# CliffKai/BridgeLang

Hardware: AMD Instinct MI355X
Metric: action-seqs/sec (7-DoF, 224px) openvla-7b bf16 (higher is better)
Workload: dtype bf16; 1 GPU; openvla-7b bf16 inference (BASELINE configs[1]): batch 16 synthetic 224px frames + 32-token prompts per GPU, predict_action = vision towers + projector + Llama prefill S=288 + 6 cached decode steps, greedy; 7 batches in flight: per step one batch is submitted (vision+prefill) while decode iteration g of the batch submitted g steps earlier, g = 1..6, runs as ONE merged 96-row pass over the weights ; batch_per_gpu=16, prompt_len=32, seq_len=288, replicas=1, hip_graph=True, pipeline_depth=7

## Files before the change

### bridgelang_amd/csrc/gemm_bf16.hip

```cpp
#include "gemm_common.h"
#include <stdlib.h>

namespace bl_gemm_bf16_impl {
using namespace blgemm;

typedef __attribute__((ext_vector_type(4))) short s16x4_t;

template <int EPI>
__global__ __launch_bounds__(256) void gemm128_kernel(GemmArgs p) {
#if defined(__HIP_DEVICE_COMPILE__)
  constexpr int BM = 128, BN = 128, WN = 2, NWAVE = 4;
  constexpr int TM = 64, TN = 64, MT = 4, NT = 4;
  constexpr int A_BYTES = BM * ROW_BYTES, BUF_BYTES = A_BYTES + BN * ROW_BYTES;
  extern __shared__ __attribute__((aligned(16))) char smem[];

  int tm, tn;
  tile_coords(p, tm, tn);
  const int m0 = tm * BM, n0 = tn * BN;
  const int tid = threadIdx.x, lane = tid & 63;
  const int wave = __builtin_amdgcn_readfirstlane(tid >> 6);
  const int wm = wave / WN, wn = wave % WN;
  const int kt32 = p.K >> 5;

  const unsigned a_bytes = (unsigned)min((long)p.M * p.lda * 2, 0xffffffffL);
// ... 382 lines not shown
        }
      }
    }
    asm volatile("s_waitcnt lgkmcnt(0)" ::: "memory");
    __builtin_amdgcn_s_barrier();
  }
#undef BL_STAGE
#undef BL_WAIT_TILES
  if constexpr (SK > 0) {
    float* slab = p.slab + (long)blockIdx.y * p.M * p.N;
#pragma unroll
    for (int i = 0; i < NB; ++i)
#pragma unroll
      for (int j = 0; j < MB; ++j) {
        const int m = wave * 16 * MB + j * 16 + l15, n = n0 + i * 16 + lg * 4;
        if (gridDim.y == 1) epilogue_store4<EPI>(p, m, n, acc[i][j]);
        else if (m < p.M && n < p.N) *(f32x4_t*)(slab + (long)m * p.N + n) = acc[i][j];
      }
    return;
  }
  if (p.splitk > 1) {
    float* slab = p.slab + (long)blockIdx.y * p.M * p.N;
#pragma unroll
    for (int i = 0; i < NB; ++i)
#pragma unroll
      for (int j = 0; j < MB; ++j) {
        const int m = wave * 16 * MB + j * 16 + l15, n = n0 + i * 16 + lg * 4;
        if (m < p.M && n < p.N) *(f32x4_t*)(slab + (long)m * p.N + n) = acc[i][j];
      }
    return;
  }
#pragma unroll
  for (int i = 0; i < NB; ++i)
#pragma unroll
    for (int j = 0; j < MB; ++j)
      epilogue_store4<EPI>(p, wave * 16 * MB + j * 16 + l15, n0 + i * 16 + lg * 4, acc[i][j]);
#endif
}

template <int EPI, int NWV, int SK>
__global__ __launch_bounds__(NWV * 64) void gemm_rows_stream_kernel(GemmArgs p, int n_tiles) {
#if defined(__HIP_DEVICE_COMPILE__)
  constexpr int MR = 6, GS = 4, NWB = 4;
  constexpr int KT_BYTES = MR * 16 * ROW_BYTES, XBUF = 2 * KT_BYTES;
  constexpr int XP = 24 / NWV, OPS = XP + GS;
  static_assert(24 % NWV == 0 && XP <= GS, "the chunk's 24 LDS-DMA pieces are dealt evenly to the waves, one per k-step");
  constexpr int LV = SK >= 8 ? 3 : SK >= 4 ? 2 : SK >= 2 ? 1 : 0;
  extern __shared__ __attribute__((aligned(16))) char smem[];
  const int tid = threadIdx.x, lane = tid & 63;
  const int wave = __builtin_amdgcn_readfirstlane(tid >> 6);
  const int l15 = lane & 15, lg = lane >> 4;
  const int tile_raw = (int)blockIdx.x * NWV + wave;
  const bool live = tile_raw < n_tiles;
  const int tile = live ? tile_raw : n_tiles - 1;
  const int kt32 = p.K >> 5;
  const int ks0 = (int)blockIdx.y * SK * p.fold_ks, nks = SK * p.fold_ks;
  const int NC = (nks + GS - 1) / GS;

  const unsigned a_bytes = (unsigned)min((long)p.M * p.lda * 2, 0xffffffffL);
  const __amdgpu_buffer_rsrc_t rsA = __builtin_amdgcn_make_buffer_rsrc((void*)p.A, 0, a_bytes, 0x00020000);
  const int prow = lane >> 3, pchunk = (lane & 7) ^ prow;
  unsigned voffA[XP];
  int ldsA[XP];
#pragma unroll
  for (int j = 0; j < XP; ++j) {
    const int q = j * NWV + wave, kt = q / 12, rb = q - kt * 12;
    voffA[j] = (unsigned)(((long)(rb * 8 + prow) * p.lda) * 2 + kt * 128 + pchunk * 16);
    ldsA[j] = kt * KT_BYTES + rb * 1024;
  }
  const u32x4_t* wbase = (const u32x4_t*)p.W + ((long)tile * kt32 + ks0) * 64 + lane;
  u32x4_t wbuf[NWB][GS];

#define BL_RS_ISSUE_PART(SLOT, C, J)                                                                          \
  do {                                                                                                        \
    const int cc__ = min((C), NC - 1);                                                                        \
    if ((J) < XP) BL_GLDS(rsA, smem + (SLOT) * XBUF + ldsA[(J) < XP ? (J) : 0], voffA[(J) < XP ? (J) : 0], (ks0 + cc__ * GS) * 64); \
    wbuf[SLOT][J] = __builtin_nontemporal_load(wbase + (long)min(cc__ * GS + (J), nks - 1) * 64);             \
  } while (0)
#define BL_RS_READX(DST, XB, S)                                                                               \
  do {                                                                                                        \
    const char* xs__ = (XB) + ((S) >> 1) * KT_BYTES + offA + ((c0 ^ (((S) & 1) * 4)) << 4);                    \
    _Pragma("unroll") for (int j = 0; j < MR; ++j) DST[j] = *(const bf16x8_t*)(xs__ + j * 16 * ROW_BYTES);    \
  } while (0)
#define BL_RS_FOLD_LEVEL(L)                                                                \
  if constexpr (LV > L) {                                                                   \
    if (!parked) {                                                                          \
      if (!((sl >> L) & 1)) {                                                               \
        _Pragma("unroll") for (int j = 0; j < MR; ++j) hold[L][j] = acc[j];                 \
        parked = true;                                                                      \
      } else {                                                                              \
        _Pragma("unroll") for (int j = 0; j < MR; ++j) acc[j] = hold[L][j] + acc[j];        \
      }                                                                                     \
    }                                                                                       \
  }
#define BL_RS_CHUNK(SLOT, C)                                                                                  \
  {                                                                                                           \
    asm volatile("s_waitcnt vmcnt(%0)" ::"n"(2 * OPS) : "memory");                                            \
    __builtin_amdgcn_s_barrier();                                                                             \
    const char* xb = smem + (SLOT) * XBUF;                                                                    \
    bf16x8_t xf[2][MR];                                                                                       \
    BL_RS_READX(xf[0], xb, 0);                                                                                \
    _Pragma("unroll") for (int s2 = 0; s2 < GS; ++s2) {                                                       \
      if (s2 + 1 < GS) BL_RS_READX(xf[(s2 + 1) & 1], xb, s2 + 1);                                             \
      __builtin_amdgcn_sched_barrier(0);    \
      const int kidx = (C) * GS + s2;                                                                         \
      if (kidx < nks) {                                                                                       \
        const bf16x8_t wf = __builtin_bit_cast(bf16x8_t, wbuf[SLOT][s2]);                                     \
        _Pragma("unroll") for (int j = 0; j < MR; ++j)                                                        \
          acc[j] = __builtin_amdgcn_mfma_f32_16x16x32_bf16(wf, xf[s2 & 1][j], acc[j], 0, 0, 0);               \
        if (SK > 1 && s2 == GS - 1 && kidx + 1 == fold_next) {           \
          bool parked = false;                                                                                \
              \
          _Pragma("unroll") for (int j = 0; j < MR; ++j) asm volatile("" : "+v"(acc[j]));                     \
          BL_RS_FOLD_LEVEL(0) BL_RS_FOLD_LEVEL(1) BL_RS_FOLD_LEVEL(2)                                         \
          if (parked) {                                                                                       \
            _Pragma("unroll") for (int j = 0; j < MR; ++j) acc[j] = (f32x4_t){0.f, 0.f, 0.f, 0.f};            \
          }                                                                                                   \
          fold_next += p.fold_ks;                                                                             \
          ++sl;                                                                                               \
        }                                                                                                     \
      }                                                                                                       \
      __builtin_amdgcn_sched_barrier(0);                                                                      \
      BL_RS_ISSUE_PART(((SLOT) + NWB - 1) % NWB, (C) + NWB - 1, s2);                                          \
      __builtin_amdgcn_sched_barrier(0);                                                                      \
    }                                                                                                         \
    asm volatile("s_waitcnt lgkmcnt(0)" ::: "memory");                                                        \
  }

  const int c0 = lg ^ (lane & 7);
  const int offA = l15 * ROW_BYTES;
  f32x4_t acc[MR], hold[LV ? LV : 1][MR];
#pragma unroll
  for (int j = 0; j < MR; ++j) acc[j] = (f32x4_t){0.f, 0.f, 0.f, 0.f};
  int fold_next = p.fold_ks, sl = 0;

#pragma unroll
  for (int c = 0; c < NWB - 1; ++c) {
#pragma unroll
    for (int j = 0; j < GS; ++j) BL_RS_ISSUE_PART(c, c, j);
    __builtin_amdgcn_sched_barrier(0);
  }
  for (int cb = 0; cb < NC; cb += NWB) {
    BL_RS_CHUNK(0, cb)
    BL_RS_CHUNK(1, cb + 1)
    BL_RS_CHUNK(2, cb + 2)
    BL_RS_CHUNK(3, cb + 3)
  }
#undef BL_RS_CHUNK
#undef BL_RS_FOLD_LEVEL
#undef BL_RS_READX
#undef BL_RS_ISSUE_PART
  if (!live) return;
  float* slab = p.slab + (long)blockIdx.y * p.M * p.N;
#pragma unroll
  for (int j = 0; j < MR; ++j) {
    const int m = j * 16 + l15, n = tile * 16 + lg * 4;
    if (gridDim.y == 1) epilogue_store4<EPI>(p, m, n, acc[j]);
    else if (m < p.M) *(f32x4_t*)(slab + (long)m * p.N + n) = acc[j];
  }
#endif
}

template <int EPI, int NT, int NST = 3>
__global__ __launch_bounds__(256) void gemm_mid2_kernel(GemmArgs p) {
#if defined(__HIP_DEVICE_COMPILE__)
  constexpr int BM = 160, BN = 32 * NT, MT = 5, LPS = 5 + NT;
  constexpr int A_BYTES = BM * ROW_BYTES, BUF_BYTES = A_BYTES + NT * 4096;
  extern __shared__ __attribute__((aligned(16))) char smem[];
  const int n0 = blockIdx.x * BN, m0 = blockIdx.y * BM;
  const int tid = threadIdx.x, lane = tid & 63;
  const int wave = __builtin_amdgcn_readfirstlane(tid >> 6);
  const int wm = wave >> 1, wn = wave & 1;
  const int kt32 = p.K >> 5;

  const unsigned a_bytes = (unsigned)min((long)p.M * p.lda * 2, 0xffffffffL);
  const unsigned w_bytes = (unsigned)min((long)p.N * p.K * 2, 0xffffffffL);
  const __amdgpu_buffer_rsrc_t rsA = __builtin_amdgcn_make_buffer_rsrc((void*)p.A, 0, a_bytes, 0x00020000);
  const __amdgpu_buffer_rsrc_t rsW = __builtin_amdgcn_make_buffer_rsrc((void*)p.W, 0, w_bytes, 0x00020000);

  const int prow = lane >> 3, pchunk = (lane & 7) ^ prow;
  unsigned voffA[MT];
#pragma unroll
  for (int j = 0; j < MT; ++j) voffA[j] = (unsigned)(((long)(m0 + (j * 4 + wave) * 8 + prow) * p.lda) * 2 + pchunk * 16);
  unsigned voffW[NT];
#pragma unroll
  for (int j = 0; j < NT; ++j) {
    const int blk = j * 4 + wave;
    voffW[j] = (unsigned)(((long)(n0 / 16 + (blk >> 1)) * kt32 + (blk & 1)) * 1024 + lane * 16);
  }

#define BL_STAGE(BUF, KT)                                                                                   \
  do {                                                                                                      \
    char* base__ = smem + (BUF) * BUF_BYTES;                                                                \
    _Pragma("unroll") for (int j = 0; j < MT; ++j) BL_GLDS(rsA, base__ + (j * 4 + wave) * 1024, voffA[j], (KT) * 128); \
    _Pragma("unroll") for (int j = 0; j < NT; ++j) BL_GLDS(rsW, base__ + A_BYTES + (j * 4 + wave) * 1024, voffW[j], (KT) * 2048); \
  } while (0)

  const int l15 = lane & 15, lg = lane >> 4;
  const int c0 = lg ^ (lane & 7);
  const int offA = (wm * 80 + l15) * ROW_BYTES;
  const int offW = A_BYTES + (wn * NT) * 2048 + lane * 16;

  f32x4_t acc[NT][MT];
#pragma unroll
  for (int i = 0; i < NT; ++i)
#pragma unroll
    for (int j = 0; j < MT; ++j) acc[i][j] = (f32x4_t){0.f, 0.f, 0.f, 0.f};

  const int nk = p.K / BK;
  static_assert(NST == 2 || NST == 3, "ring depth");
  BL_STAGE(0, 0);
  if (NST == 3 && 1 < nk) BL_STAGE(1, 1);
  for (int kt = 0; kt < nk; ++kt) {
    if (kt + NST - 1 < nk) BL_STAGE((kt + NST - 1) % NST, kt + NST - 1);
    const int later = min(NST - 1, nk - 1 - kt);
    if (later == 2) asm volatile("s_waitcnt vmcnt(%0)" ::"n"(2 * LPS) : "memory");
    else if (later == 1) asm volatile("s_waitcnt vmcnt(%0)" ::"n"(LPS) : "memory");
    else asm volatile("s_waitcnt vmcnt(0)" ::: "memory");
    __builtin_amdgcn_s_barrier();
    const char* base = smem + (kt % NST) * BUF_BYTES;
#pragma unroll
    for (int ks = 0; ks < 2; ++ks) {
      const int cb = (c0 ^ (ks * 4)) << 4;
      bf16x8_t wf[NT], af[MT];
#pragma unroll
      for (int i = 0; i < NT; ++i) wf[i] = *(const bf16x8_t*)(base + offW + i * 2048 + ks * 1024);
#pragma unroll
      for (int j = 0; j < MT; ++j) af[j] = *(const bf16x8_t*)(base + offA + j * 16 * ROW_BYTES + cb);
#pragma unroll
      for (int i = 0; i < NT; ++i)
#pragma unroll
        for (int j = 0; j < MT; ++j) acc[i][j] = __builtin_amdgcn_mfma_f32_16x16x32_bf16(wf[i], af[j], acc[i][j], 0, 0, 0);
    }
    asm volatile("s_waitcnt lgkmcnt(0)" ::: "memory");
    __builtin_amdgcn_s_barrier();
  }
#undef BL_STAGE
#pragma unroll
  for (int i = 0; i < NT; ++i)
#pragma unroll
    for (int j = 0; j < MT; ++j)
      epilogue_store4<EPI>(p, m0 + wm * 80 + j * 16 + l15, n0 + (wn * NT + i) * 16 + lg * 4, acc[i][j]);
#endif
}

template <int EPI>
__global__ __launch_bounds__(512) void gemm288s_kernel(GemmArgs p) {
#if defined(__HIP_DEVICE_COMPILE__)
  constexpr int BM = 288, BN = 256;
  constexpr int A_BYTES = BM * ROW_BYTES, DUMMY = A_BYTES, W_OFF = A_BYTES + 4096, STAGE = W_OFF + 32768;
  extern __shared__ __attribute__((aligned(16))) char smem[];
  int tm, tn;
  tile_coords(p, tm, tn);
  const int m0 = tm * BM, n0 = tn * BN;
  const int tid = threadIdx.x, lane = tid & 63;
  const int wave = __builtin_amdgcn_readfirstlane(tid >> 6);
  const int wm = wave >> 2, wn = wave & 3;
  const int l15 = lane & 15, lg = lane >> 4;
  const int kt32 = p.K >> 5, nk = p.K / BK;

  const unsigned a_bytes = (unsigned)min((long)p.M * p.lda * 2, 0xffffffffL);
  const unsigned w_bytes = (unsigned)min((long)p.N * p.K * 2, 0xffffffffL);
  const int prow = lane >> 3, pchunk = (lane & 7) ^ prow;
  unsigned voffA[5];
  int ldsA[5];
#pragma unroll
  for (int j = 0; j < 5; ++j) {
    const int pi = wave + 8 * j;
    voffA[j] = (unsigned)(((long)(m0 + pi * 8 + prow) * p.lda) * 2 + pchunk * 16);
    ldsA[j] = pi < 36 ? pi * 1024 : DUMMY + (pi - 36) * 1024;
  }
  const unsigned a4_bytes = wave < 4 ? a_bytes : 0u;
  unsigned voffW[2];
#pragma unroll
  for (int q = 0; q < 2; ++q) voffW[q] = (unsigned)((long)(n0 / 16 + 2 * wave + q) * kt32 * 1024 + lane * 16);
  const int ldsW = W_OFF + 2 * wave * 2048;
#define BL_RS(PTR, BYTES) __builtin_amdgcn_make_buffer_rsrc((void*)(PTR), 0, (BYTES), 0x00020000)
#define ISSUE_A(J, TILE)                                                                                  \
  do {                                                                                                    \
    const int t__ = (TILE);                                                                               \
    const __amdgpu_buffer_rsrc_t rs__ = BL_RS(p.A, t__ < nk ? ((J) < 4 ? a_bytes : a4_bytes) : 0u);       \
    BL_GLDS(rs__, smem + (t__ & 1) * STAGE + ldsA[J], voffA[J], t__ * 128);                               \
  } while (0)
#define ISSUE_W(Q, KS, TILE)                                                                              \
  do {                                                                                                    \
    const int t__ = (TILE);                                                                               \
    const __amdgpu_buffer_rsrc_t rs__ = BL_RS(p.W, t__ < nk ? w_bytes : 0u);                              \
    BL_GLDS(rs__, smem + (t__ & 1) * STAGE + ldsW + (Q) * 2048 + (KS) * 1024, voffW[Q] + (KS) * 1024, t__ * 2048); \
  } while (0)
  const int cb0 = (lg ^ (lane & 7)) << 4;
  const int offX = (wm * 144 + l15) * ROW_BYTES;
  const int offY = W_OFF + wn * 8192 + lane * 16;
#define READ_X(T3, SB)                                                                                    \
  _Pragma("unroll") for (int i = 0; i < 3; ++i) {                                                         \
    X[i * 2] = *(const bf16x8_t*)((SB) + offX + (3 * (T3) + i) * 2048 + cb0);                             \
    X[i * 2 + 1] = *(const bf16x8_t*)((SB) + offX + (3 * (T3) + i) * 2048 + (cb0 ^ 64));                  \
  }
#define READ_Y(DST, NH, SB)                                                                               \
  _Pragma("unroll") for (int j = 0; j < 2; ++j) {                                                         \
    DST[j * 2] = *(const bf16x8_t*)((SB) + offY + (2 * (NH) + j) * 2048);                                 \
    DST[j * 2 + 1] = *(const bf16x8_t*)((SB) + offY + (2 * (NH) + j) * 2048 + 1024);                      \
  }
#define MMA(YR, T3, NH)                                                                                   \
  do {                                                                                                    \
    __builtin_amdgcn_s_setprio(1);                                                                        \
    _Pragma("unroll") for (int ks = 0; ks < 2; ++ks)                                                      \
      _Pragma("unroll") for (int j = 0; j < 2; ++j)                                                       \
        _Pragma("unroll") for (int i = 0; i < 3; ++i)                                                     \
          acc[2 * (NH) + j][3 * (T3) + i] = __builtin_amdgcn_mfma_f32_16x16x32_bf16(                      \
              YR[j * 2 + ks], X[i * 2 + ks], acc[2 * (NH) + j][3 * (T3) + i], 0, 0, 0);                   \
    __builtin_amdgcn_s_setprio(0);                                                                        \
  } while (0)
#define BAR()                                                                                             \
  do {                                                                                                    \
    __builtin_amdgcn_s_barrier();                                                                         \
    __builtin_amdgcn_sched_barrier(0);                                                                    \
  } while (0)
#define WAIT_LGKM() asm volatile("s_waitcnt lgkmcnt(0)" ::: "memory")
#define WAIT_VM2_LGKM() asm volatile("s_waitcnt vmcnt(2) lgkmcnt(0)" ::: "memory")
#define SLOT1(SC, T) do { READ_X(0, SC); READ_Y(Ya, 0, SC); __builtin_amdgcn_sched_barrier(0); ISSUE_A(2, (T) + 1); WAIT_LGKM(); } while (0)
#define SLOT2(SC, T) do { READ_Y(Yb, 1, SC); __builtin_amdgcn_sched_barrier(0); ISSUE_A(3, (T) + 1); ISSUE_A(4, (T) + 1); WAIT_LGKM(); } while (0)
#define SLOT3(SC, T) do { READ_X(1, SC); __builtin_amdgcn_sched_barrier(0); ISSUE_W(0, 0, (T) + 1); WAIT_LGKM(); } while (0)
#define SLOT4(SC, T) do { ISSUE_W(0, 1, (T) + 1); ISSUE_W(1, 0, (T) + 1); } while (0)
#define SLOT5(SC, T) do { READ_X(2, SC); __builtin_amdgcn_sched_barrier(0); ISSUE_W(1, 1, (T) + 1); WAIT_LGKM(); } while (0)
#define SLOT6(SC, T) do { ISSUE_A(0, (T) + 2); ISSUE_A(1, (T) + 2); WAIT_VM2_LGKM(); } while (0)
#define BL_EPILOGUE()                                                                                     \
  do {                                                                                                    \
    asm volatile("s_waitcnt vmcnt(0)" ::: "memory");                                                      \
    const int ncol__[4] = {n0 + wn * 64 + lg * 4, n0 + wn * 64 + 16 + lg * 4, n0 + wn * 64 + 32 + lg * 4,      \
                           n0 + wn * 64 + 48 + lg * 4};                                                   \
    epilogue_tile<EPI, 4, 9>(p, m0 + wm * 144 + l15, ncol__, m0 + 288, n0 + 256, acc);                    \
  } while (0)

  f32x4_t acc[4][9];
#pragma unroll
  for (int i = 0; i < 4; ++i)
#pragma unroll
    for (int j = 0; j < 9; ++j) acc[i][j] = (f32x4_t){0.f, 0.f, 0.f, 0.f};
  bf16x8_t X[6], Ya[4], Yb[4];
  char* const S0 = smem;
  char* const S1 = smem + STAGE;

  ISSUE_A(0, 0); ISSUE_A(1, 0); ISSUE_A(2, 0); ISSUE_A(3, 0); ISSUE_A(4, 0);
  ISSUE_W(0, 0, 0); ISSUE_W(0, 1, 0); ISSUE_W(1, 0, 0); ISSUE_W(1, 1, 0);
  ISSUE_A(0, 1); ISSUE_A(1, 1);
  asm volatile("s_waitcnt vmcnt(2)" ::: "memory");
  BAR();
  if (wm == 0) {
    SLOT1(S0, 0);
    BAR();
    for (int t = 0; t < nk; t += 2) {
      MMA(Ya, 0, 0); BAR();   SLOT2(S0, t); BAR();
      MMA(Yb, 0, 1); BAR();   SLOT3(S0, t); BAR();
      MMA(Yb, 1, 1); BAR();   SLOT4(S0, t); BAR();
      MMA(Ya, 1, 0); BAR();   SLOT5(S0, t); BAR();
      MMA(Ya, 2, 0); BAR();   SLOT6(S0, t); BAR();
      MMA(Yb, 2, 1); BAR();   SLOT1(S1, t + 1); BAR();
      MMA(Ya, 0, 0); BAR();   SLOT2(S1, t + 1); BAR();
      MMA(Yb, 0, 1); BAR();   SLOT3(S1, t + 1); BAR();
      MMA(Yb, 1, 1); BAR();   SLOT4(S1, t + 1); BAR();
      MMA(Ya, 1, 0); BAR();   SLOT5(S1, t + 1); BAR();
      MMA(Ya, 2, 0); BAR();   SLOT6(S1, t + 1); BAR();
      MMA(Yb, 2, 1); BAR();   SLOT1(S0, t + 2); BAR();
    }
    BL_EPILOGUE();
    return;
  }
  BAR();
  for (int t = 0; t < nk; t += 2) {
    SLOT1(S0, t); BAR();       MMA(Ya, 0, 0); BAR();
    SLOT2(S0, t); BAR();       MMA(Yb, 0, 1); BAR();
    SLOT3(S0, t); BAR();       MMA(Yb, 1, 1); BAR();
    SLOT4(S0, t); BAR();       MMA(Ya, 1, 0); BAR();
    SLOT5(S0, t); BAR();       MMA(Ya, 2, 0); BAR();
    SLOT6(S0, t); BAR();       MMA(Yb, 2, 1); BAR();
    SLOT1(S1, t + 1); BAR();   MMA(Ya, 0, 0); BAR();
    SLOT2(S1, t + 1); BAR();   MMA(Yb, 0, 1); BAR();
    SLOT3(S1, t + 1); BAR();   MMA(Yb, 1, 1); BAR();
    SLOT4(S1, t + 1); BAR();   MMA(Ya, 1, 0); BAR();
    SLOT5(S1, t + 1); BAR();   MMA(Ya, 2, 0); BAR();
    SLOT6(S1, t + 1); BAR();   MMA(Yb, 2, 1); BAR();
  }
  BL_EPILOGUE();
#undef BL_RS
#undef ISSUE_A
#undef ISSUE_W
#undef READ_X
#undef READ_Y
#undef MMA
#undef BAR
#undef WAIT_LGKM
#undef WAIT_VM2_LGKM
#undef SLOT1
#undef SLOT2
#undef SLOT3
#undef SLOT4
#undef SLOT5
#undef SLOT6
#undef BL_EPILOGUE
#endif
}

template <int EPI, bool TN = false>
__global__ __launch_bounds__(512) void gemm256s_kernel(GemmArgs p) {
#if defined(__HIP_DEVICE_COMPILE__)
  constexpr int BM = 256, BN = 256;
  constexpr int STAGE = 65536, W_OFF = 32768;
  extern __shared__ __attribute__((aligned(16))) char smem[];

  int tm, tn;
  const int nk_all = TN ? (p.K + BK - 1) / BK : p.K / BK;
  int kt_begin = 0, nk = nk_all;
  const int ptiles = p.splitk > 1 ? 0 : p.ptiles;
  int vb = blockIdx.x;
  if (p.splitk > 1) {
    lin_to_tile(p, p.tail_base + blockIdx.x / p.splitk, tm, tn);
    const int slice = blockIdx.x % p.splitk;
    kt_begin = (int)(((long)slice * nk_all) / p.splitk) & ~1;
    nk = slice + 1 == p.splitk ? nk_all : ((int)(((long)(slice + 1) * nk_all) / p.splitk) & ~1);
  } else if (ptiles > 0) {
    tile_coords_v(p, vb, ptiles, tm, tn);
  } else {
    tile_coords(p, tm, tn);
  }
  int m0 = tm * BM, n0 = tn * BN;
  const int tid = threadIdx.x, lane = tid & 63;
  const int wave = __builtin_amdgcn_readfirstlane(tid >> 6);
  const int wm = wave >> 2, wn = wave & 3;
  const int l15 = lane & 15, lg = lane >> 4;
  const int kt32 = p.K >> 5;

  const long a_total = TN ? ((long)(p.K - 1) * p.lda + p.M) * 2 : (long)p.M * p.lda * 2;
  const long w_total = TN ? ((long)(p.K - 1) * p.ldw + p.N) * 2 : (long)p.N * p.K * 2;
  const int kstepX = TN ? (int)(64 * p.lda * 2) : 128, kstepY = TN ? (int)(64 * p.ldw * 2) : 2048;
#define TILE_A_OFF(M0) (TN ? (long)(M0) * 2 : (long)(M0) * p.lda * 2)
#define TILE_W_OFF(N0) (TN ? (long)(N0) * 2 : (long)((N0) / 16) * (p.K >> 5) * 1024)
  const char* Acur = (const char*)p.A + TILE_A_OFF(m0);
  const char* Wcur = (const char*)p.W + TILE_W_OFF(n0);
  unsigned a_bytes = (unsigned)min(a_total - TILE_A_OFF(m0), 0xffffffffL);
  unsigned w_bytes = (unsigned)min(w_total - TILE_W_OFF(n0), 0xffffffffL);
  const char* Anext = Acur; const char* Wnext = Wcur;
  unsigned a_bytes_next = 0u, w_bytes_next = 0u;
  int m0_next = 0, n0_next = 0;
#define BL_NEXT_TILE()                                                                      \
  do {                                                                                      \
    a_bytes_next = 0u; w_bytes_next = 0u;                                                   \
    if (ptiles > 0 && vb + (int)gridDim.x < ptiles) {                                       \
      int tm__, tn__;                                                                       \
      tile_coords_v(p, vb + (int)gridDim.x, ptiles, tm__, tn__);                            \
      m0_next = tm__ * BM; n0_next = tn__ * BN;                                             \
      Anext = (const char*)p.A + TILE_A_OFF(m0_next);                                       \
      Wnext = (const char*)p.W + TILE_W_OFF(n0_next);                                       \
      a_bytes_next = (unsigned)min(a_total - TILE_A_OFF(m0_next), 0xffffffffL);             \
      w_bytes_next = (unsigned)min(w_total - TILE_W_OFF(n0_next), 0xffffffffL);             \
    }                                                                                       \
  } while (0)
  BL_NEXT_TILE();

  const int prow = lane >> 3, pchunk = (lane & 7) ^ prow;
  unsigned voffX[2][2], voffY[2][2];
  int ldsX[2][2], ldsY[2];
  if constexpr (!TN) {
#pragma unroll
    for (int mh = 0; mh < 2; ++mh)
#pragma unroll
      for (int j = 0; j < 2; ++j) {
        const int pi = 2 * wave + j, row0 = (pi >> 3) * 128 + mh * 64 + (pi & 7) * 8;
        voffX[mh][j] = (unsigned)(((long)(row0 + prow) * p.lda) * 2 + pchunk * 16);
        ldsX[mh][j] = row0 * ROW_BYTES;
      }
#pragma unroll
    for (int nh = 0; nh < 2; ++nh) {
      const int nt = (wave >> 1) * 4 + 2 * nh + (wave & 1);
      voffY[nh][0] = (unsigned)((long)nt * kt32 * 1024 + lane * 16);
      voffY[nh][1] = voffY[nh][0] + 1024;
      ldsY[nh] = W_OFF + nt * 2048;
    }
  } else {
#pragma unroll
    for (int mh = 0; mh < 2; ++mh)
#pragma unroll
      for (int j = 0; j < 2; ++j) {
        const int pi = 2 * wave + j, t = (pi & 7) * 8 + prow, pos = lane & 7;
        const int c = ((((pos >> 1) ^ ((t >> 1) & 3)) << 1) | (pos & 1));
        voffX[mh][j] = (unsigned)((long)t * p.lda * 2 + (long)((pi >> 3) * 128 + mh * 64) * 2 + c * 16);
        ldsX[mh][j] = ((pi >> 3) * 128 + mh * 64 + (pi & 7) * 8) * ROW_BYTES;
      }
#pragma unroll
    for (int nh = 0; nh < 2; ++nh) {
#pragma unroll
      for (int j = 0; j < 2; ++j) {
        const int t = (2 * wave + j) * 4 + (lane >> 4), pos = lane & 15;
        const int c = ((((pos >> 1) ^ (t & 7)) << 1) | (pos & 1));
        voffY[nh][j] = (unsigned)((long)t * p.ldw * 2 + (long)(nh * 128) * 2 + c * 16);
      }
      ldsY[nh] = W_OFF + nh * 16384 + wave * 2048;
    }
  }
#define BL_RS(PTR, BYTES) __builtin_amdgcn_make_buffer_rsrc((void*)(PTR), 0, (BYTES), 0x00020000)
#define ISSUE_X(MH, TILE)                                                                   \
  do {                                                                                      \
    const int t__ = (TILE);                                                                 \
    const bool nx__ = t__ >= nk;                         \
    const int tt__ = nx__ ? t__ - nk : t__;                                                 \
    const __amdgpu_buffer_rsrc_t rs__ = BL_RS(nx__ ? Anext : Acur, nx__ ? a_bytes_next : a_bytes); \
    char* b__ = smem + (t__ & 1) * STAGE;                                                   \
    BL_GLDS(rs__, b__ + ldsX[MH][0], voffX[MH][0], tt__ * kstepX);                             \
    BL_GLDS(rs__, b__ + ldsX[MH][1], voffX[MH][1], tt__ * kstepX);                             \
  } while (0)
#define ISSUE_Y(NH, TILE)                                                                   \
  do {                                                                                      \
    const int t__ = (TILE);                                                                 \
    const bool nx__ = t__ >= nk;                                                            \
    const int tt__ = nx__ ? t__ - nk : t__;                                                 \
    const __amdgpu_buffer_rsrc_t rs__ = BL_RS(nx__ ? Wnext : Wcur, nx__ ? w_bytes_next : w_bytes); \
    char* b__ = smem + (t__ & 1) * STAGE;                                                   \
    BL_GLDS(rs__, b__ + ldsY[NH], voffY[NH][0], tt__ * kstepY);                               \
    BL_GLDS(rs__, b__ + ldsY[NH] + 1024, voffY[NH][1], tt__ * kstepY);                        \
  } while (0)
  const int cb0 = (lg ^ (lane & 7)) << 4;
  const int offX = (wm * 128 + l15) * ROW_BYTES;
  const int offY = W_OFF + wn * 8192 + lane * 16;
  const int trX = (wm * 128) * ROW_BYTES + (4 * lg + (l15 >> 2)) * 128 + (l15 & 3) * 8, swX = ((lg & 1) << 1) | (l15 >> 3);
  const int trY = W_OFF + (4 * lg + (l15 >> 2)) * 256 + (l15 & 3) * 8, swY = ((lg & 1) << 2) | (l15 >> 2);
  const unsigned ldsbase = (unsigned)(size_t)LDS_PTR(smem);
#define BL_TR(DST, ADDR, OFF) asm volatile("ds_read_b64_tr_b16 %0, %1 offset:%2" : "=v"(DST) : "v"(ADDR), "n"(OFF))
#define BL_PIN(R) asm volatile("" : "+v"(R))
#define READ_X(DST, MH, SB)                                                                             \
  do {                                                                                                  \
    if constexpr (!TN) {                                                                                \
      _Pragma("unroll") for (int i = 0; i < 4; ++i) {                                                   \
        DST[i * 2] = *(const bf16x8_t*)((SB) + offX + (MH) * 8192 + i * 2048 + cb0);                    \
        DST[i * 2 + 1] = *(const bf16x8_t*)((SB) + offX + (MH) * 8192 + i * 2048 + (cb0 ^ 64));        \
      }                                                                                                 \
    } else {                                                                                            \
      _Pragma("unroll") for (int i = 0; i < 4; ++i) {                                                   \
        const unsigned a__ = ldsbase + (unsigned)((SB) - smem) + trX + ((i ^ swX) << 5);                \
        BL_TR(DST##2[i * 4 + 0], a__, (MH) * 8192);                                                     \
        BL_TR(DST##2[i * 4 + 1], a__, (MH) * 8192 + 2048);                                              \
        BL_TR(DST##2[i * 4 + 2], a__, (MH) * 8192 + 4096);                                              \
        BL_TR(DST##2[i * 4 + 3], a__, (MH) * 8192 + 4096 + 2048);                                       \
      }                                                                                                 \
    }                                                                                                   \
  } while (0)
#define READ_Y(DST, NH, SB)                                                                             \
  do {                                                                                                  \
    if constexpr (!TN) {                                                                                \
      _Pragma("unroll") for (int j = 0; j < 2; ++j) {                                                   \
        DST[j * 2] = *(const bf16x8_t*)((SB) + offY + (2 * (NH) + j) * 2048);                           \
        DST[j * 2 + 1] = *(const bf16x8_t*)((SB) + offY + (2 * (NH) + j) * 2048 + 1024);                \
      }                                                                                                 \
    } else {                                                                                            \
      _Pragma("unroll") for (int j = 0; j < 2; ++j) {                                                   \
        const unsigned a__ = ldsbase + (unsigned)((SB) - smem) + trY + (((wn * 2 + j) ^ swY) << 5);     \
        BL_TR(DST##2[j * 4 + 0], a__, (NH) * 16384);                                                    \
        BL_TR(DST##2[j * 4 + 1], a__, (NH) * 16384 + 4096);                                             \
        BL_TR(DST##2[j * 4 + 2], a__, (NH) * 16384 + 8192);                                             \
        BL_TR(DST##2[j * 4 + 3], a__, (NH) * 16384 + 8192 + 4096);                                      \
      }                                                                                                 \
    }                                                                                                   \
  } while (0)
#define BL_FRAG(R2, F, KS)                                                                              \
  __builtin_bit_cast(bf16x8_t, ((u32x4_t){R2[(F) * 4 + 2 * (KS)][0], R2[(F) * 4 + 2 * (KS)][1],         \
                                          R2[(F) * 4 + 2 * (KS) + 1][0], R2[(F) * 4 + 2 * (KS) + 1][1]}))
#define MMA(XR, YR, MH, NH)                                                                             \
  do {                                                                                                  \
    if constexpr (TN) {                                                                                 \
      _Pragma("unroll") for (int q = 0; q < 16; ++q) BL_PIN(XR##2[q]);                                  \
      _Pragma("unroll") for (int q = 0; q < 8; ++q) BL_PIN(YR##2[q]);                                   \
    }                                                                                                   \
    __builtin_amdgcn_s_setprio(1);                                                                      \
    _Pragma("unroll") for (int ks = 0; ks < 2; ++ks)                                                    \
      _Pragma("unroll") for (int j = 0; j < 2; ++j)                                                     \
        _Pragma("unroll") for (int i = 0; i < 4; ++i) {                                                 \
          if constexpr (TN)                                                                             \
            acc[2 * (NH) + j][4 * (MH) + i] = __builtin_amdgcn_mfma_f32_16x16x32_bf16(                  \
                BL_FRAG(YR##2, j, ks), BL_FRAG(XR##2, i, ks), acc[2 * (NH) + j][4 * (MH) + i], 0, 0, 0); \
          else                                                                                          \
            acc[2 * (NH) + j][4 * (MH) + i] = __builtin_amdgcn_mfma_f32_16x16x32_bf16(                  \
                YR[j * 2 + ks], XR[i * 2 + ks], acc[2 * (NH) + j][4 * (MH) + i], 0, 0, 0);              \
        }                                                                                               \
    __builtin_amdgcn_s_setprio(0);                                                                      \
  } while (0)
#define BAR()                                   \
  do {                                          \
    __builtin_amdgcn_s_barrier();               \
    __builtin_amdgcn_sched_barrier(0);          \
  } while (0)
#define WAIT_VM8() asm volatile("s_waitcnt vmcnt(8)" ::: "memory")
#define WAIT_VM10_LGKM() asm volatile("s_waitcnt vmcnt(10) lgkmcnt(0)" ::: "memory")
#define WAIT_LGKM() asm volatile("s_waitcnt lgkmcnt(0)" ::: "memory")
#define ISSUE_READ(I, R) do { R; __builtin_amdgcn_sched_barrier(0); I; } while (0)
#define ISSUE_Q0(T) ISSUE_X(1, (T) + 1)
#define ISSUE_Q1(T) ISSUE_Y(0, (T) + 2)
#define ISSUE_Q2(T) ISSUE_X(0, (T) + 2)
#define ISSUE_Q3(T) ISSUE_Y(1, (T) + 2)
#define BL_EPILOGUE()                                                                                     \
  do {                                                                                                    \
    if (a_bytes_next == 0u && w_bytes_next == 0u)    \
      asm volatile("s_waitcnt vmcnt(0)" ::: "memory");                                                    \
    if (p.splitk > 1) {                                                                                   \
      long off__ = ((long)blockIdx.x * 32 * 512 + tid) * 4;                                               \
      asm volatile("" : "+v"(off__));    \
      float* dst = p.slab + off__;                                                                        \
      _Pragma("unroll") for (int i = 0; i < 4; ++i)                                                       \
        _Pragma("unroll") for (int j = 0; j < 8; ++j) *(f32x4_t*)(dst + (long)(i * 8 + j) * 512 * 4) = acc[i][j]; \
    } else {                                                                                              \
      int ncol__[4];                                                                                      \
      _Pragma("unroll") for (int i = 0; i < 4; ++i)                                                       \
        ncol__[i] = TN ? n0 + (i >> 1) * 128 + wn * 32 + (i & 1) * 16 + lg * 4 : n0 + wn * 64 + i * 16 + lg * 4; \
      epilogue_tile<EPI, 4, 8>(p, m0 + wm * 128 + l15, ncol__, m0 + 256, n0 + 256, acc);                  \
    }                                                                                                     \
  } while (0)

#define BL_ADVANCE()                                                                                      \
  do {                                                                                                    \
    vb += (int)gridDim.x;                                                                                 \
    m0 = m0_next; n0 = n0_next; Acur = Anext; Wcur = Wnext; a_bytes = a_bytes_next; w_bytes = w_bytes_next; \
    BL_NEXT_TILE();                                                                                       \
    _Pragma("unroll") for (int i = 0; i < 4; ++i)                                                         \
      _Pragma("unroll") for (int j = 0; j < 8; ++j) acc[i][j] = (f32x4_t){0.f, 0.f, 0.f, 0.f};            \
  } while (0)

  f32x4_t acc[4][8];
#pragma unroll
  for (int i = 0; i < 4; ++i)
#pragma unroll
    for (int j = 0; j < 8; ++j) acc[i][j] = (f32x4_t){0.f, 0.f, 0.f, 0.f};
  bf16x8_t X[8], Ya[4], Yb[4];
  u32x2_t X2[16], Ya2[8], Yb2[8];
  char* const S0 = smem;
  char* const S1 = smem + STAGE;
  const int t0 = kt_begin;

  ISSUE_Y(0, t0); ISSUE_X(0, t0); ISSUE_Y(1, t0); ISSUE_X(1, t0); ISSUE_Y(0, t0 + 1); ISSUE_X(0, t0 + 1); ISSUE_Y(1, t0 + 1);
  asm volatile("s_waitcnt vmcnt(10)" ::: "memory");
  BAR();
  READ_Y(Ya, 0, S0);

  if (wm == 0) {
    READ_X(X, 0, S0);
    WAIT_LGKM();
    BAR();
    for (;;) {
    for (int t = t0; t < nk; t += 2) {
      MMA(X, Ya, 0, 0); WAIT_VM8(); BAR();   ISSUE_READ(ISSUE_Q0(t), READ_Y(Yb, 1, S0)); WAIT_LGKM(); BAR();
      MMA(X, Yb, 0, 1); WAIT_VM8(); BAR();   ISSUE_READ(ISSUE_Q1(t), READ_X(X, 1, S0));  WAIT_LGKM(); BAR();
      MMA(X, Yb, 1, 1); WAIT_VM8(); BAR();   ISSUE_READ(ISSUE_Q2(t), READ_Y(Yb, 0, S1)); WAIT_LGKM(); BAR();
      MMA(X, Ya, 1, 0); WAIT_VM8(); BAR();   ISSUE_READ(ISSUE_Q3(t), READ_X(X, 0, S1));  WAIT_LGKM(); BAR();
      MMA(X, Yb, 0, 0); WAIT_VM8(); BAR();   ISSUE_READ(ISSUE_Q0(t + 1), READ_Y(Ya, 1, S1)); WAIT_LGKM(); BAR();
      MMA(X, Ya, 0, 1); WAIT_VM8(); BAR();   ISSUE_READ(ISSUE_Q1(t + 1), READ_X(X, 1, S1));  WAIT_LGKM(); BAR();
      MMA(X, Ya, 1, 1); WAIT_VM8(); BAR();   ISSUE_READ(ISSUE_Q2(t + 1), READ_Y(Ya, 0, S0)); WAIT_LGKM(); BAR();
      MMA(X, Yb, 1, 0); WAIT_VM8(); BAR();   ISSUE_READ(ISSUE_Q3(t + 1), READ_X(X, 0, S0));  WAIT_LGKM(); BAR();
    }
    const bool more = a_bytes_next != 0u;
    BL_EPILOGUE();
    if (!more) break;
    BL_ADVANCE();
    }
    return;
  }
  WAIT_LGKM();
  BAR();
  for (;;) {
  for (int t = t0; t < nk; t += 2) {
    ISSUE_READ(ISSUE_Q0(t), READ_X(X, 0, S0));  WAIT_VM10_LGKM(); BAR();   MMA(X, Ya, 0, 0); BAR();
    ISSUE_READ(ISSUE_Q1(t), READ_Y(Yb, 1, S0)); WAIT_VM10_LGKM(); BAR();   MMA(X, Yb, 0, 1); BAR();
    ISSUE_READ(ISSUE_Q2(t), READ_X(X, 1, S0));  WAIT_VM10_LGKM(); BAR();   MMA(X, Yb, 1, 1); BAR();
    ISSUE_READ(ISSUE_Q3(t), READ_Y(Yb, 0, S1)); WAIT_VM10_LGKM(); BAR();   MMA(X, Ya, 1, 0); BAR();
    ISSUE_READ(ISSUE_Q0(t + 1), READ_X(X, 0, S1));  WAIT_VM10_LGKM(); BAR();   MMA(X, Yb, 0, 0); BAR();
    ISSUE_READ(ISSUE_Q1(t + 1), READ_Y(Ya, 1, S1)); WAIT_VM10_LGKM(); BAR();   MMA(X, Ya, 0, 1); BAR();
    ISSUE_READ(ISSUE_Q2(t + 1), READ_X(X, 1, S1));  WAIT_VM10_LGKM(); BAR();   MMA(X, Ya, 1, 1); BAR();
    ISSUE_READ(ISSUE_Q3(t + 1), READ_Y(Ya, 0, S0)); WAIT_VM10_LGKM(); BAR();   MMA(X, Yb, 1, 0); BAR();
  }
  const bool more = a_bytes_next != 0u;
  BL_EPILOGUE();
  if (!more) break;
  BL_ADVANCE();
  }
#undef BL_EPILOGUE
#undef BL_ADVANCE
#undef BL_NEXT_TILE
#undef TILE_A_OFF
#undef TILE_W_OFF
#undef ISSUE_X
#undef ISSUE_Y
#undef READ_X
#undef READ_Y
#undef BL_TR
#undef BL_PIN
#undef BL_FRAG
#undef MMA
#undef BAR
#undef WAIT_VM8
#undef WAIT_VM10_LGKM
#undef WAIT_LGKM
#undef ISSUE_READ
#undef ISSUE_Q0
#undef ISSUE_Q1
#undef ISSUE_Q2
#undef ISSUE_Q3
// ... 87 lines not shown
```

Baseline: 269.9 action-seqs/s.

## Restructure 288-row GEMM ping-pong into three phases with weights prefetched two tiles ahead

Reorganizes the wave-specialized ping-pong GEMM loop (288-row tile) from six slots per k-tile into three phases. Each phase now runs both Y halves' MFMAs back-to-back, which halves the number of barriers per k-tile. The schedule also changes: weight tiles are now prefetched two k-tiles ahead and activation tiles one ahead, with vmcnt(4) waits replacing vmcnt(2). This targets barrier overhead and weight-load latency in the merged decode GEMM. In exchange, all Y registers are live at once, which raises register pressure, and each phase is longer, which may reduce overlap between the two wave groups.

```diff
diff --git a/bridgelang_amd/csrc/gemm_bf16.hip b/bridgelang_amd/csrc/gemm_bf16.hip
--- a/bridgelang_amd/csrc/gemm_bf16.hip
+++ b/bridgelang_amd/csrc/gemm_bf16.hip
@@ -708,13 +708,16 @@
     DST[j * 2 + 1] = *(const bf16x8_t*)((SB) + offY + (2 * (NH) + j) * 2048 + 1024);                      \
   }
 #define MMA(YR, T3, NH)                                                                                   \
+  _Pragma("unroll") for (int ks = 0; ks < 2; ++ks)                                                        \
+    _Pragma("unroll") for (int j = 0; j < 2; ++j)                                                         \
+      _Pragma("unroll") for (int i = 0; i < 3; ++i)                                                       \
+        acc[2 * (NH) + j][3 * (T3) + i] = __builtin_amdgcn_mfma_f32_16x16x32_bf16(                        \
+            YR[j * 2 + ks], X[i * 2 + ks], acc[2 * (NH) + j][3 * (T3) + i], 0, 0, 0);
+#define PHASE(T3)                                                                                         \
   do {                                                                                                    \
     __builtin_amdgcn_s_setprio(1);                                                                        \
-    _Pragma("unroll") for (int ks = 0; ks < 2; ++ks)                                                      \
-      _Pragma("unroll") for (int j = 0; j < 2; ++j)                                                       \
-        _Pragma("unroll") for (int i = 0; i < 3; ++i)                                                     \
-          acc[2 * (NH) + j][3 * (T3) + i] = __builtin_amdgcn_mfma_f32_16x16x32_bf16(                      \
-              YR[j * 2 + ks], X[i * 2 + ks], acc[2 * (NH) + j][3 * (T3) + i], 0, 0, 0);                   \
+    MMA(Ya, T3, 0)                                                                                        \
+    MMA(Yb, T3, 1)                                                                                        \
     __builtin_amdgcn_s_setprio(0);                                                                        \
   } while (0)
 #define BAR()                                                                                             \
@@ -723,13 +726,10 @@
     __builtin_amdgcn_sched_barrier(0);                                                                    \
   } while (0)
 #define WAIT_LGKM() asm volatile("s_waitcnt lgkmcnt(0)" ::: "memory")
-#define WAIT_VM2_LGKM() asm volatile("s_waitcnt vmcnt(2) lgkmcnt(0)" ::: "memory")
-#define SLOT1(SC, T) do { READ_X(0, SC); READ_Y(Ya, 0, SC); __builtin_amdgcn_sched_barrier(0); ISSUE_A(2, (T) + 1); WAIT_LGKM(); } while (0)
-#define SLOT2(SC, T) do { READ_Y(Yb, 1, SC); __builtin_amdgcn_sched_barrier(0); ISSUE_A(3, (T) + 1); ISSUE_A(4, (T) + 1); WAIT_LGKM(); } while (0)
-#define SLOT3(SC, T) do { READ_X(1, SC); __builtin_amdgcn_sched_barrier(0); ISSUE_W(0, 0, (T) + 1); WAIT_LGKM(); } while (0)
-#define SLOT4(SC, T) do { ISSUE_W(0, 1, (T) + 1); ISSUE_W(1, 0, (T) + 1); } while (0)
-#define SLOT5(SC, T) do { READ_X(2, SC); __builtin_amdgcn_sched_barrier(0); ISSUE_W(1, 1, (T) + 1); WAIT_LGKM(); } while (0)
-#define SLOT6(SC, T) do { ISSUE_A(0, (T) + 2); ISSUE_A(1, (T) + 2); WAIT_VM2_LGKM(); } while (0)
+#define WAIT_VM4_LGKM() asm volatile("s_waitcnt vmcnt(4) lgkmcnt(0)" ::: "memory")
+#define SLOT0(SC, T) do { READ_X(0, SC); READ_Y(Ya, 0, SC); READ_Y(Yb, 1, SC); __builtin_amdgcn_sched_barrier(0); ISSUE_A(0, (T) + 1); ISSUE_A(1, (T) + 1); WAIT_LGKM(); } while (0)
+#define SLOT1(SC, T) do { READ_X(1, SC); __builtin_amdgcn_sched_barrier(0); ISSUE_A(2, (T) + 1); ISSUE_A(3, (T) + 1); ISSUE_A(4, (T) + 1); WAIT_LGKM(); } while (0)
+#define SLOT2(SC, T) do { READ_X(2, SC); __builtin_amdgcn_sched_barrier(0); ISSUE_W(0, 0, (T) + 2); ISSUE_W(0, 1, (T) + 2); ISSUE_W(1, 0, (T) + 2); ISSUE_W(1, 1, (T) + 2); WAIT_VM4_LGKM(); } while (0)
 #define BL_EPILOGUE()                                                                                     \
   do {                                                                                                    \
     asm volatile("s_waitcnt vmcnt(0)" ::: "memory");                                                      \
@@ -749,43 +749,31 @@
 
   ISSUE_A(0, 0); ISSUE_A(1, 0); ISSUE_A(2, 0); ISSUE_A(3, 0); ISSUE_A(4, 0);
   ISSUE_W(0, 0, 0); ISSUE_W(0, 1, 0); ISSUE_W(1, 0, 0); ISSUE_W(1, 1, 0);
-  ISSUE_A(0, 1); ISSUE_A(1, 1);
-  asm volatile("s_waitcnt vmcnt(2)" ::: "memory");
+  ISSUE_W(0, 0, 1); ISSUE_W(0, 1, 1); ISSUE_W(1, 0, 1); ISSUE_W(1, 1, 1);
+  asm volatile("s_waitcnt vmcnt(4)" ::: "memory");
   BAR();
   if (wm == 0) {
-    SLOT1(S0, 0);
+    SLOT0(S0, 0);
     BAR();
     for (int t = 0; t < nk; t += 2) {
-      MMA(Ya, 0, 0); BAR();   SLOT2(S0, t); BAR();
-      MMA(Yb, 0, 1); BAR();   SLOT3(S0, t); BAR();
-      MMA(Yb, 1, 1); BAR();   SLOT4(S0, t); BAR();
-      MMA(Ya, 1, 0); BAR();   SLOT5(S0, t); BAR();
-      MMA(Ya, 2, 0); BAR();   SLOT6(S0, t); BAR();
-      MMA(Yb, 2, 1); BAR();   SLOT1(S1, t + 1); BAR();
-      MMA(Ya, 0, 0); BAR();   SLOT2(S1, t + 1); BAR();
-      MMA(Yb, 0, 1); BAR();   SLOT3(S1, t + 1); BAR();
-      MMA(Yb, 1, 1); BAR();   SLOT4(S1, t + 1); BAR();
-      MMA(Ya, 1, 0); BAR();   SLOT5(S1, t + 1); BAR();
-      MMA(Ya, 2, 0); BAR();   SLOT6(S1, t + 1); BAR();
-      MMA(Yb, 2, 1); BAR();   SLOT1(S0, t + 2); BAR();
+      PHASE(0); BAR();   SLOT1(S0, t); BAR();
+      PHASE(1); BAR();   SLOT2(S0, t); BAR();
+      PHASE(2); BAR();   SLOT0(S1, t + 1); BAR();
+      PHASE(0); BAR();   SLOT1(S1, t + 1); BAR();
+      PHASE(1); BAR();   SLOT2(S1, t + 1); BAR();
+      PHASE(2); BAR();   SLOT0(S0, t + 2); BAR();
     }
     BL_EPILOGUE();
     return;
   }
   BAR();
   for (int t = 0; t < nk; t += 2) {
-    SLOT1(S0, t); BAR();       MMA(Ya, 0, 0); BAR();
-    SLOT2(S0, t); BAR();       MMA(Yb, 0, 1); BAR();
-    SLOT3(S0, t); BAR();       MMA(Yb, 1, 1); BAR();
-    SLOT4(S0, t); BAR();       MMA(Ya, 1, 0); BAR();
-    SLOT5(S0, t); BAR();       MMA(Ya, 2, 0); BAR();
-    SLOT6(S0, t); BAR();       MMA(Yb, 2, 1); BAR();
-    SLOT1(S1, t + 1); BAR();   MMA(Ya, 0, 0); BAR();
-    SLOT2(S1, t + 1); BAR();   MMA(Yb, 0, 1); BAR();
-    SLOT3(S1, t + 1); BAR();   MMA(Yb, 1, 1); BAR();
-    SLOT4(S1, t + 1); BAR();   MMA(Ya, 1, 0); BAR();
-    SLOT5(S1, t + 1); BAR();   MMA(Ya, 2, 0); BAR();
-    SLOT6(S1, t + 1); BAR();   MMA(Yb, 2, 1); BAR();
+    SLOT0(S0, t); BAR();       PHASE(0); BAR();
+    SLOT1(S0, t); BAR();       PHASE(1); BAR();
+    SLOT2(S0, t); BAR();       PHASE(2); BAR();
+    SLOT0(S1, t + 1); BAR();   PHASE(0); BAR();
+    SLOT1(S1, t + 1); BAR();   PHASE(1); BAR();
+    SLOT2(S1, t + 1); BAR();   PHASE(2); BAR();
   }
   BL_EPILOGUE();
 #undef BL_RS
@@ -794,15 +782,13 @@
 #undef READ_X
 #undef READ_Y
 #undef MMA
+#undef PHASE
 #undef BAR
 #undef WAIT_LGKM
-#undef WAIT_VM2_LGKM
+#undef WAIT_VM4_LGKM
+#undef SLOT0
 #undef SLOT1
 #undef SLOT2
-#undef SLOT3
-#undef SLOT4
-#undef SLOT5
-#undef SLOT6
 #undef BL_EPILOGUE
 #endif
 }
```

Result: faster. 276.6 action-seqs/s (median of 6 runs) (+2.5%).
